# vsergeev/luaradio

Hardware: NVIDIA H100
Metric: WBFM-mono chain Msamples/s (input samples) @N H100; FIR-128 HBM GB/s vs roofline (higher is better)
Workload: dtype f32

## Files before the change

luaradio_b200/csrc/common.cuh:

```cuda
#pragma once
#include <cuda_runtime.h>
#include <stdint.h>
#include <stddef.h>
#include <atomic>
#include <math.h>

namespace lrb {

#define LRB_MAX_DEVICES 16

struct Ctx {
    int device = -1;
    int sm_count = 132;
    cudaStream_t stream = nullptr;
    bool own_stream = false;
    std::atomic<uint64_t> launches{0};
    int reserve_ctas = 0;
    long long lead_samples = 0;
    cudaEvent_t lead_event = nullptr;
    cudaStream_t side = nullptr;
    cudaEvent_t ev_fork = nullptr, ev_join = nullptr;
};
Ctx& ctx();
void set_error(const char* fmt, ...);
bool cuda_ok(cudaError_t e, const char* what);

#define LRB_CHECK(call)                                   \
    do {                                                  \
        if (!::lrb::cuda_ok((call), #call)) return -1;    \
    } while (0)

inline uint64_t turns_to_fix(double turns) {
    long double t = (long double)turns;
    t -= floorl(t);
    long double f = ldexpl(t, 64);
    if (f >= 18446744073709551616.0L) return 0;
    return (uint64_t)f;
}

constexpr size_t SIDE_STREAM_MIN = (size_t)1 << 18;
cudaStream_t side_fork(cudaStream_t s);
void side_join(cudaStream_t s, cudaStream_t side);

inline void count_launch(int n = 1) { ctx().launches.fetch_add((uint64_t)n, std::memory_order_relaxed); }

enum FirKind { FIR_CRCF = 0, FIR_CCCF = 1, FIR_RRRF = 2, FIR_HILBERT = 3 };

int launch_fir_generic(FirKind kind, const void* x, const void* hist, const void* taps, int M, int D,
                       long long first, long long n_out, void* y, cudaStream_t s);
int launch_hist_update(const void* x, long long n, const void* hist_old, void* hist_new, int H,
                       int elem_size, cudaStream_t s);

bool poly_generic_supports(FirKind kind, int M, int D);
int launch_poly_generic(FirKind kind, const void* x, const void* hist, const void* taps_host, int M, int D,
                        long long first, long long n, long long n_out, void* y, cudaStream_t s);

int launch_rotator(const float2* x, float2* y, long long n, uint64_t turns_fix, uint64_t g0, cudaStream_t s);
int launch_discrim(const float2* x, const float2* prev, float* y, long long n, float inv_gain, cudaStream_t s);
int launch_downsample(const void* x, void* y, long long first, long long n_out, int D, int elem_size, cudaStream_t s);
int launch_cmag(const float2* x, float* y, long long n, cudaStream_t s);
int launch_c2r(const float2* x, float* y, long long n, cudaStream_t s);
int launch_copy_last(const void* x, long long n, void* dst, int elem_size, cudaStream_t s);
int launch_zero_segments(void* const* ptrs, const size_t* bytes, int count, cudaStream_t s);

struct IirScanWork {
    int* ticket = nullptr;
    int* flags = nullptr;
    void* agg = nullptr;
    void* pfx = nullptr;
    int max_tiles = 0;
    unsigned epoch = 0;
};
int iir_work_alloc(IirScanWork* w, int elem_size);
void iir_work_free(IirScanWork* w);
long long iir_max_per_launch(const IirScanWork& w);
int launch_iir1(bool complex_data, const void* x, long long n, void* y, const float* b_host, int nb, float c,
                const void* xhist_in, void* xhist_out, const void* ystate_in, void* ystate_out,
                long long first, int D, IirScanWork* w, cudaStream_t s);

int launch_iir_general(bool complex_data, const void* x, long long n, void* y, const float* b, int nb, const float* a, int na,
                       const void* xhist, const void* yhist, long long warm, cudaStream_t s);

int launch_synth_white(float2* dst, uint64_t n0, long long n, uint32_t seed, cudaStream_t s);
int launch_synth_fm(float2* dst, uint64_t n0, long long n, uint32_t seed, double rate, double carrier,
                    double deviation, float amp, float noise, cudaStream_t s);

#ifdef __CUDACC__
__device__ __forceinline__ float2 ffma2(float2 a, float2 b, float2 c) {
    return make_float2(__fmaf_rn(a.x, b.x, c.x), __fmaf_rn(a.y, b.y, c.y));
}
__device__ __forceinline__ float2 fmul2(float2 a, float2 b) { return make_float2(__fmul_rn(a.x, b.x), __fmul_rn(a.y, b.y)); }
__device__ __forceinline__ float2 fadd2(float2 a, float2 b) { return make_float2(__fadd_rn(a.x, b.x), __fadd_rn(a.y, b.y)); }
__device__ __forceinline__ float2 phasor_from_fix(uint64_t ph) {
    int t = (int)(uint32_t)(ph >> 32);
    float half_turns = (float)t * 4.656612873077393e-10f;
    float s, c;
    sincospif(half_turns, &s, &c);
    return make_float2(c, s);
}
__device__ __forceinline__ float fast_atan2f(float y, float x) {
    const float ax = fabsf(x), ay = fabsf(y);
    const float mx = fmaxf(ax, ay), mn = fminf(ax, ay);
    const float a = mx > 0.f ? __fdividef(mn, mx) : 0.f;
    const float z = a * a;
    float r = 0.0028340641874819994f;
    r = fmaf(r, z, -0.016005029901862144f);
    r = fmaf(r, z, 0.042587608098983765f);
    r = fmaf(r, z, -0.07495445758104324f);
    r = fmaf(r, z, 0.10636754333972931f);
    r = fmaf(r, z, -0.14202570915222168f);
    r = fmaf(r, z, 0.19992484152317047f);
    r = fmaf(r, z, -0.3333306610584259f);
    r = fmaf(r, z, 1.0f);
    r *= a;
    r = ay > ax ? 1.57079632679489662f - r : r;
    r = x < 0.f ? 3.14159265358979324f - r : r;
    return copysignf(r, y);
}
__device__ __forceinline__ float2 fast_atan2f_x2(float2 y, float2 x) {
    const float ax0 = fabsf(x.x), ay0 = fabsf(y.x), ax1 = fabsf(x.y), ay1 = fabsf(y.y);
    const float mx0 = fmaxf(ax0, ay0), mn0 = fminf(ax0, ay0), mx1 = fmaxf(ax1, ay1), mn1 = fminf(ax1, ay1);
    const float2 a = make_float2(mx0 > 0.f ? __fdividef(mn0, mx0) : 0.f, mx1 > 0.f ? __fdividef(mn1, mx1) : 0.f);
    const float2 z = fmul2(a, a);
    float2 r = make_float2(0.0028340641874819994f, 0.0028340641874819994f);
    r = ffma2(r, z, make_float2(-0.016005029901862144f, -0.016005029901862144f));
    r = ffma2(r, z, make_float2(0.042587608098983765f, 0.042587608098983765f));
    r = ffma2(r, z, make_float2(-0.07495445758104324f, -0.07495445758104324f));
    r = ffma2(r, z, make_float2(0.10636754333972931f, 0.10636754333972931f));
    r = ffma2(r, z, make_float2(-0.14202570915222168f, -0.14202570915222168f));
    r = ffma2(r, z, make_float2(0.19992484152317047f, 0.19992484152317047f));
    r = ffma2(r, z, make_float2(-0.3333306610584259f, -0.3333306610584259f));
    r = ffma2(r, z, make_float2(1.0f, 1.0f));
    r = fmul2(r, a);
    float r0 = ay0 > ax0 ? 1.57079632679489662f - r.x : r.x;
    float r1 = ay1 > ax1 ? 1.57079632679489662f - r.y : r.y;
    r0 = x.x < 0.f ? 3.14159265358979324f - r0 : r0;
    r1 = x.y < 0.f ? 3.14159265358979324f - r1 : r1;
    return make_float2(copysignf(r0, y.x), copysignf(r1, y.y));
}
__device__ __forceinline__ float2 cmul(float2 a, float2 b) {
    float2 t = fmul2(make_float2(-a.y, a.x), make_float2(b.y, b.y));
    return ffma2(a, make_float2(b.x, b.x), t);
}
#endif

}
```

luaradio_b200/csrc/tuner.cu:

```cuda
#include "common.cuh"
#include "blocks.h"

#include <cmath>
#include <cstdlib>
#include <cstring>
#include <new>
#include <string>
#include <type_traits>
#include <vector>

namespace lrb {

namespace {

#ifndef LRB_PT_THREADS
#define LRB_PT_THREADS 64
#define LRB_PT_R 8
#define LRB_PT_CTAS 8
#define LRB_PT_PREFETCH 9
#define LRB_PT_BATCH 7
#endif
#ifndef LRB_PT_EXPERIMENT
#define LRB_PT_EXPERIMENT 0
#endif
#ifndef LRB_PT_EARLY_REST
#define LRB_PT_EARLY_REST 0
#endif
constexpr int PT_THREADS = LRB_PT_THREADS;
constexpr int PT_R = LRB_PT_R;
constexpr int PT_TO = PT_THREADS * PT_R;
constexpr int PT_MAXTAPS = 144;
constexpr int PT_BATCH = LRB_PT_BATCH;

constexpr int PT_MAXIT = 48;
struct PolyParams {
    float hr[PT_MAXTAPS];
    float2 step[PT_MAXIT];
    uint64_t turns_fix;
    uint64_t g0;
    long long off;
    int M;
    float pole_c;
    float pole_cp[6];
};
constexpr int PT_POLE_WARM = (64 % LRB_PT_R == 0) ? 64 : ((72 % LRB_PT_R == 0) ? 72 : 4 * LRB_PT_R);
static_assert(PT_POLE_WARM % LRB_PT_R == 0 && PT_POLE_WARM % 4 == 0 && PT_POLE_WARM >= 64, "pole warm-up must cover whole threads");

template <int D, int Q>
struct PolyShape {
    static constexpr int RD = PT_R * D;
    static constexpr int T = Q * D + 1;
    static constexpr int SPAN = (PT_TO + Q - 1) * D + 1;
    static constexpr int PAIRS = (SPAN + 1) / 2;
    static constexpr int ITERS = (PAIRS + PT_THREADS - 1) / PT_THREADS;
    static constexpr int LOADED = 2 * ITERS * PT_THREADS;
    __host__ __device__ static constexpr int pad(int e) { return e + 2 * (e / RD); }
    static constexpr int ELEMS = LOADED + 2 * (LOADED / RD) + 2;
    static constexpr size_t SMEM = (size_t)ELEMS * sizeof(float2);
    static constexpr int RAW = ELEMS;
    static constexpr size_t SMEM_BULK = (size_t)(ELEMS + LOADED) * sizeof(float2);
    static constexpr int NSEG = (LOADED + RD - 1) / RD;
    static constexpr int PPS = RD / 2;
    static constexpr int RG = PT_THREADS / PPS;
    static constexpr int RITERS = (NSEG + RG - 1) / RG;
};

__device__ __forceinline__ uint32_t smem_addr(const void* p) { return (uint32_t)__cvta_generic_to_shared(p); }
__device__ __forceinline__ void mbar_init(uint64_t* bar) {
    asm volatile("mbarrier.init.shared::cta.b64 [%0], 1;\n\tfence.mbarrier_init.release.cluster;\n\t"
                 "fence.proxy.async.shared::cta;" :: "r"(smem_addr(bar)) : "memory");
}
__device__ __forceinline__ void mbar_expect_tx(uint64_t* bar, uint32_t bytes) {
    asm volatile("mbarrier.arrive.expect_tx.shared::cta.b64 _, [%0], %1;" :: "r"(smem_addr(bar)), "r"(bytes) : "memory");
}
__device__ __forceinline__ void mbar_wait(uint64_t* bar, uint32_t parity) {
    asm volatile("{\n\t.reg .pred p;\n\tLRB_WAIT_%=:\n\t"
                 "mbarrier.try_wait.parity.shared::cta.b64 p, [%0], %1;\n\t"
                 "@!p bra LRB_WAIT_%=;\n\t}" :: "r"(smem_addr(bar)), "r"(parity) : "memory");
}
__device__ __forceinline__ void fence_proxy_async() { asm volatile("fence.proxy.async.shared::cta;" ::: "memory"); }
__device__ __forceinline__ void bulk_g2s(void* dst, const void* src, uint32_t bytes, uint64_t* bar) {
    asm volatile("cp.async.bulk.shared::cluster.global.mbarrier::complete_tx::bytes [%0], [%1], %2, [%3];"
                 :: "r"(smem_addr(dst)), "l"(src), "r"(bytes), "r"(smem_addr(bar)) : "memory");
}

template <int B, int E, typename F>
__device__ __forceinline__ void static_for(F&& f) {
    if constexpr (B < E) {
        f(std::integral_constant<int, B>{});
        static_for<B + 1, E>(f);
    }
}

constexpr int DISC_OV = 4;
template <bool DISC>
struct TileStride { static constexpr int TS = DISC ? PT_TO - DISC_OV : PT_TO; };

template <int D, int Q, bool ROT, bool DISC, bool EDGE, bool REAL = false, bool POLE = false>
__global__ void __launch_bounds__(PT_THREADS, LRB_PT_CTAS)
polyphase_crcf_kernel(const float2* __restrict__ x, const float2* __restrict__ hist, long long n,
                      void* __restrict__ yv, long long n_out, const __grid_constant__ PolyParams P,
                      long long t_lo, long long t_hi,
                      const float2* __restrict__ prev_in, float2* __restrict__ prev_out, float inv_gain) {
    using S = PolyShape<D, Q>;
    static_assert(!(REAL && (ROT || DISC)), "the real-stream variant has no translator / discriminator");
    static_assert(REAL || !POLE, "the fused pole exists in the real-stream variant only");
    constexpr int PW = POLE ? PT_POLE_WARM : 0;
    constexpr int PAY = PT_TO - PW;
    constexpr int TS = REAL ? 2 * PAY : TileStride<DISC>::TS;
    constexpr int NPRE = S::ITERS < LRB_PT_PREFETCH ? S::ITERS : LRB_PT_PREFETCH;
    constexpr int LANE1 = PAY * D;
    const float* __restrict__ xr = reinterpret_cast<const float*>(x);
    const float* __restrict__ histr = reinterpret_cast<const float*>(hist);
    extern __shared__ __align__(16) float2 smem[];
    __shared__ float2 s_edge[PT_THREADS / 32];
    const int tid = threadIdx.x, lane = tid & 31, warp = tid >> 5;
    const int Hm1 = P.M - 1;

    constexpr bool BULK = !EDGE && !REAL && DISC;
    __shared__ __align__(8) uint64_t s_bar;
    uint32_t bar_phase = 0;

    float2 A0 = make_float2(1.f, 0.f), A1 = make_float2(1.f, 0.f);
    const int rg = tid / S::PPS, rw = tid - rg * S::PPS;
    constexpr int NE0 = (BULK && ROT) ? S::RITERS : 1;
    float2 E0[NE0];
    float2 W1 = make_float2(1.f, 0.f);
    if constexpr (BULK && ROT) {
        W1 = phasor_from_fix(P.turns_fix);
#pragma unroll
        for (int it = 0; it < NE0; ++it)
            E0[it] = phasor_from_fix(P.turns_fix * (uint64_t)((rg + S::RG * it) * S::RD + 2 * rw));
    } else if constexpr (ROT) {
        A0 = phasor_from_fix(P.turns_fix * (uint64_t)(2 * tid));
        A1 = phasor_from_fix(P.turns_fix * (uint64_t)(2 * tid + 1));
    }
    const bool rot_last = rg < S::RG && (rg + S::RG * (S::RITERS - 1)) * S::RD + 2 * rw < S::LOADED;
    auto tile_of = [&](long long idx) -> long long { return EDGE ? (idx < t_lo ? idx : t_hi + (idx - t_lo)) : (t_lo + idx); };
    const long long n_work = EDGE ? 0 : (t_hi - t_lo);
    long long widx = blockIdx.x;

    auto issue_tile = [&](long long idx) {
        if (tid == 0) {
            fence_proxy_async();
            mbar_expect_tx(&s_bar, (uint32_t)(S::LOADED * sizeof(float2)));
            bulk_g2s(smem + S::RAW, x + (P.off + tile_of(idx) * (long long)(TS * D)), (uint32_t)(S::LOADED * sizeof(float2)), &s_bar);
        }
    };
    if constexpr (BULK) {
        if (tid == 0) mbar_init(&s_bar);
        __syncthreads();
        if (widx < n_work) issue_tile(widx);
    }

    auto ld_pair = [&](long long Bt, int k) -> float4 {
        if constexpr (REAL) {
            const float2* pa = reinterpret_cast<const float2*>(xr + Bt) + (tid + k * PT_THREADS);
            const float2 a = __ldcs(pa), b = __ldcs(pa + LANE1 / 2);
            return make_float4(a.x, b.x, a.y, b.y);
        } else {
            return __ldcs(reinterpret_cast<const float4*>(x + Bt) + (tid + k * PT_THREADS));
        }
    };
    float4 pre[NPRE];
    constexpr int REST = (S::ITERS - NPRE) < PT_BATCH ? (S::ITERS - NPRE) : PT_BATCH;
    float4 rest[REST > 0 ? REST : 1];
    if constexpr (!EDGE && !BULK) {
        if (widx < n_work) {
            const long long Bt = P.off + tile_of(widx) * (long long)(TS * D);
#pragma unroll
            for (int k = 0; k < NPRE; ++k) pre[k] = ld_pair(Bt, k);
            if constexpr (LRB_PT_EARLY_REST) {
#pragma unroll
                for (int k = 0; k < REST; ++k) rest[k] = ld_pair(Bt, NPRE + k);
            }
        }
    }

    for (;;) {
        if constexpr (!EDGE) { if (widx >= n_work) break; }
        const long long tile = tile_of(widx);
        const long long B = P.off + tile * (long long)(TS * D);
        const long long m0 = tile * TS - (DISC ? DISC_OV : 0) - PW;

        auto stage_pair = [&](float4 v, int it) {
            const int u = tid + it * PT_THREADS;
            float2 a = make_float2(v.x, v.y), b = make_float2(v.z, v.w);
            if constexpr (ROT) {
                const float2 st = P.step[it];
                a = cmul(a, cmul(A0, st));
                b = cmul(b, cmul(A1, st));
            }
            *reinterpret_cast<float4*>(smem + S::pad(2 * u)) = make_float4(a.x, a.y, b.x, b.y);
        };
        if constexpr (BULK) {
            if (LRB_PT_EXPERIMENT != 1 || widx == blockIdx.x) {
                mbar_wait(&s_bar, bar_phase);
                bar_phase ^= 1;
                if (rg < S::RG) {
                    const float2* src = smem + S::RAW + rg * S::RD + 2 * rw;
                    float2* dst = smem + rg * (S::RD + 2) + 2 * rw;
#pragma unroll
                    for (int it = 0; it < S::RITERS; ++it) {
                        if (it == S::RITERS - 1 && !rot_last) break;
                        float4 v = *reinterpret_cast<const float4*>(src + it * S::RG * S::RD);
                        if constexpr (ROT) {
                            const float2 a = cmul(make_float2(v.x, v.y), E0[it]);
                            const float2 b = cmul(make_float2(v.z, v.w), cmul(E0[it], W1));
                            v = make_float4(a.x, a.y, b.x, b.y);
                        }
                        *reinterpret_cast<float4*>(dst + it * S::RG * (S::RD + 2)) = v;
                    }
                }
            }
        } else if constexpr (!EDGE && LRB_PT_EXPERIMENT == 1) {
            if (widx == blockIdx.x) {
#pragma unroll 1
                for (int it = 0; it < S::ITERS; ++it) stage_pair(ld_pair(B, it), it);
            }
        } else if constexpr (!EDGE) {
            if constexpr (!LRB_PT_EARLY_REST) {
#pragma unroll
                for (int k = 0; k < REST; ++k) rest[k] = ld_pair(B, NPRE + k);
            }
#pragma unroll
            for (int k = 0; k < NPRE; ++k) stage_pair(pre[k], k);
#pragma unroll
            for (int k = 0; k < REST; ++k) stage_pair(rest[k], NPRE + k);
#pragma unroll 1
            for (int it0 = NPRE + REST; it0 < S::ITERS; it0 += PT_BATCH) {
                float4 buf[PT_BATCH];
#pragma unroll
                for (int k = 0; k < PT_BATCH; ++k)
                    if (it0 + k < S::ITERS) buf[k] = ld_pair(B, it0 + k);
#pragma unroll
                for (int k = 0; k < PT_BATCH; ++k)
                    if (it0 + k < S::ITERS) stage_pair(buf[k], it0 + k);
            }
        } else {
#pragma unroll 7
            for (int it = 0; it < S::ITERS; ++it) {
                const long long i0 = B + 2LL * (tid + it * PT_THREADS);
                if constexpr (REAL) {
                    auto g = [&](long long i) -> float {
                        return (i >= 0) ? (i < n ? __ldg(xr + i) : 0.f) : ((Hm1 + i >= 0) ? __ldg(histr + (Hm1 + i)) : 0.f);
                    };
                    stage_pair(make_float4(g(i0), g(i0 + LANE1), g(i0 + 1), g(i0 + 1 + LANE1)), it);
                    continue;
                }
                const float2 a = (i0 >= 0) ? (i0 < n ? __ldg(x + i0) : make_float2(0.f, 0.f))
                                           : ((Hm1 + i0 >= 0) ? __ldg(hist + (Hm1 + i0)) : make_float2(0.f, 0.f));
                const long long i1 = i0 + 1;
                const float2 b = (i1 >= 0) ? (i1 < n ? __ldg(x + i1) : make_float2(0.f, 0.f))
                                           : ((Hm1 + i1 >= 0) ? __ldg(hist + (Hm1 + i1)) : make_float2(0.f, 0.f));
                stage_pair(make_float4(a.x, a.y, b.x, b.y), it);
            }
        }
        __syncthreads();

        if constexpr (BULK && LRB_PT_EXPERIMENT != 1) {
            if (widx + gridDim.x < n_work) issue_tile(widx + gridDim.x);
        }
        if constexpr (!EDGE && !BULK && LRB_PT_EXPERIMENT != 1) {
            const long long nidx = widx + gridDim.x;
            if (nidx < n_work) {
                const long long Bn = P.off + tile_of(nidx) * (long long)(TS * D);
#pragma unroll
                for (int k = 0; k < NPRE; ++k) pre[k] = ld_pair(Bn, k);
            }
        }

        float2 acc[PT_R];
#pragma unroll
        for (int r = 0; r < PT_R; ++r) acc[r] = make_float2(0.f, 0.f);
        const float2* tb = smem + tid * (S::RD + 2);
        static_for<0, (LRB_PT_EXPERIMENT == 2 ? 1 : PT_R + Q)>([&](auto jc) {
            constexpr int j = decltype(jc)::value;
            float2 xs[D];
            constexpr int e0 = j * D;
            if constexpr (j == PT_R + Q - 1) {
                xs[0] = tb[S::pad(e0)];
            } else {
                static_for<0, D>([&](auto pc) {
                    constexpr int pp = decltype(pc)::value;
                    constexpr int e = e0 + pp;
                    if constexpr ((e & 1) && pp >= 1) {
                    } else if constexpr (!(e & 1) && pp + 1 < D) {
                        const float4 v = *reinterpret_cast<const float4*>(tb + S::pad(e));
                        xs[pp] = make_float2(v.x, v.y);
                        xs[pp + 1] = make_float2(v.z, v.w);
                    } else {
                        xs[pp] = tb[S::pad(e)];
                    }
                });
            }
            static_for<0, PT_R>([&](auto rc) {
                constexpr int r = decltype(rc)::value;
                constexpr int qq = j - r;
                if constexpr (qq >= 0 && qq <= Q) {
                    static_for<0, D>([&](auto pc) {
                        constexpr int pp = decltype(pc)::value;
                        if constexpr (qq * D + pp < S::T) {
                            const float h = P.hr[qq * D + pp];
                            acc[r] = ffma2(xs[pp], make_float2(h, h), acc[r]);
                        }
                    });
                }
            });
        });
        if constexpr (!EDGE && !BULK && LRB_PT_EARLY_REST) {
            const long long nidx = widx + gridDim.x;
            if (nidx < n_work) {
                const long long Bn = P.off + tile_of(nidx) * (long long)(TS * D);
#pragma unroll
                for (int k = 0; k < REST; ++k) rest[k] = ld_pair(Bn, NPRE + k);
            }
        }
        if constexpr (ROT && !DISC) {
            const float2 Pt = phasor_from_fix(P.turns_fix * (P.g0 + (uint64_t)B));
#pragma unroll
            for (int r = 0; r < PT_R; ++r) acc[r] = cmul(acc[r], Pt);
        }

        const long long mbase = m0 + (long long)tid * PT_R;
        if constexpr (POLE) {
            const float c = P.pole_c;
            if (tile == 0 && tid < PW / PT_R) {
#pragma unroll
                for (int r = 0; r < PT_R; ++r) acc[r].x = 0.f;
                if (tid == PW / PT_R - 1) acc[PT_R - 1].x = __ldg(reinterpret_cast<const float*>(prev_in));
            }
#pragma unroll
            for (int r = 1; r < PT_R; ++r) acc[r] = ffma2(acc[r - 1], make_float2(c, c), acc[r]);
            float2 Bv = acc[PT_R - 1];
#pragma unroll
            for (int k = 0; k < 5; ++k) {
                const float2 o = make_float2(__shfl_up_sync(0xffffffffu, Bv.x, 1 << k), __shfl_up_sync(0xffffffffu, Bv.y, 1 << k));
                if (lane >= (1 << k)) Bv = ffma2(o, make_float2(P.pole_cp[k], P.pole_cp[k]), Bv);
            }
            if (lane == 31) s_edge[warp] = Bv;
            float2 prevB = make_float2(__shfl_up_sync(0xffffffffu, Bv.x, 1), __shfl_up_sync(0xffffffffu, Bv.y, 1));
            if (lane == 0) prevB = make_float2(0.f, 0.f);
            __syncthreads();
            float2 carryW = make_float2(0.f, 0.f);
            for (int w = 0; w < warp; ++w) carryW = ffma2(carryW, make_float2(P.pole_cp[5], P.pole_cp[5]), s_edge[w]);
            float f_lane = 1.f;
#pragma unroll
            for (int k = 0; k < 5; ++k) if (lane & (1 << k)) f_lane *= P.pole_cp[k];
            const float2 excl = ffma2(carryW, make_float2(f_lane, f_lane), prevB);
            float cpow = c;
#pragma unroll
            for (int r = 0; r < PT_R; ++r) { acc[r] = ffma2(excl, make_float2(cpow, cpow), acc[r]); cpow *= c; }
        }
        if constexpr (REAL) {
            float* y = reinterpret_cast<float*>(yv);
#pragma unroll
            for (int half = 0; half < 2; ++half) {
                const long long mb = mbase + half * PAY;
                if (POLE && tid < PW / PT_R) continue;
                float v[PT_R];
#pragma unroll
                for (int r = 0; r < PT_R; ++r) v[r] = half ? acc[r].y : acc[r].x;
                if (mb + PT_R <= n_out && ((reinterpret_cast<uintptr_t>(y + mb) & 15) == 0)) {
#pragma unroll
                    for (int r = 0; r < PT_R; r += 4)
                        __stcs(reinterpret_cast<float4*>(y + mb + r), make_float4(v[r], v[r + 1], v[r + 2], v[r + 3]));
                } else {
#pragma unroll
                    for (int r = 0; r < PT_R; ++r)
                        if (mb + r < n_out) y[mb + r] = v[r];
                }
                if constexpr (POLE) {
                    if (mb <= n_out - 1 && n_out - 1 < mb + PT_R) {
#pragma unroll
                        for (int r = 0; r < PT_R; ++r)
                            if (mb + r == n_out - 1) *reinterpret_cast<float*>(prev_out) = v[r];
                    }
                }
            }
            __syncthreads();
        } else if constexpr (!DISC) {
            float2* y = reinterpret_cast<float2*>(yv);
            if (mbase + PT_R <= n_out && ((reinterpret_cast<uintptr_t>(y + mbase) & 15) == 0)) {
                float4* y4 = reinterpret_cast<float4*>(y + mbase);
#pragma unroll
                for (int r = 0; r < PT_R; r += 2)
                    __stcs(y4 + r / 2, make_float4(acc[r].x, acc[r].y, acc[r + 1].x, acc[r + 1].y));
            } else {
#pragma unroll
                for (int r = 0; r < PT_R; ++r)
                    if (mbase + r < n_out) y[mbase + r] = acc[r];
            }
            __syncthreads();
        } else {
            float* yd = reinterpret_cast<float*>(yv);
            float2 left;
            left.x = __shfl_up_sync(0xffffffffu, acc[PT_R - 1].x, 1);
            left.y = __shfl_up_sync(0xffffffffu, acc[PT_R - 1].y, 1);
            if (lane == 31) s_edge[warp] = acc[PT_R - 1];
            __syncthreads();
            if (lane == 0 && warp > 0) left = s_edge[warp - 1];
            bool zero_prev = false;
            if (EDGE && tid == 0 && tile == 0) {
                const float2 Pt = ROT ? phasor_from_fix(P.turns_fix * (P.g0 + (uint64_t)B)) : make_float2(1.f, 0.f);
                const float2 pv = __ldg(prev_in);
                acc[DISC_OV - 1] = cmul(pv, make_float2(Pt.x, -Pt.y));
                zero_prev = pv.x == 0.f && pv.y == 0.f;
            }
            const int s0 = tid * PT_R;
            float* yt = yd + m0;
            float dout[PT_R];
#pragma unroll
            for (int r = 0; r < PT_R; r += 2) {
                const float2 c0 = acc[r], p0 = (r == 0) ? left : acc[r - 1];
                const float2 c1 = acc[r + 1], p1 = acc[r];
                const float2 t0 = ffma2(c0, make_float2(p0.x, p0.x), fmul2(make_float2(c0.y, -c0.x), make_float2(p0.y, p0.y)));
                const float2 t1 = ffma2(c1, make_float2(p1.x, p1.x), fmul2(make_float2(c1.y, -c1.x), make_float2(p1.y, p1.y)));
                const float2 ang = fast_atan2f_x2(make_float2(t0.y, t1.y), make_float2(t0.x, t1.x));
                dout[r] = ang.x * inv_gain;
                dout[r + 1] = ang.y * inv_gain;
            }
            if (EDGE && zero_prev) {
                const float2 Pt = ROT ? phasor_from_fix(P.turns_fix * (P.g0 + (uint64_t)B)) : make_float2(1.f, 0.f);
                const float2 ya = ROT ? cmul(acc[DISC_OV], Pt) : acc[DISC_OV];
                const float pz = 0.f, nz = -0.f;
                const float re = __fsub_rn(__fmul_rn(ya.x, pz), __fmul_rn(ya.y, nz));
                const float im = __fadd_rn(__fmul_rn(ya.x, nz), __fmul_rn(ya.y, pz));
                dout[DISC_OV] = atan2f(im, re) * inv_gain;
            }
            if constexpr (!EDGE) {
                if (((reinterpret_cast<uintptr_t>(yt) + DISC_OV * sizeof(float)) & 15) == 0) {
                    static_assert(DISC_OV == 4 && PT_R % 4 == 0, "thread 0 skips exactly its first float4");
#pragma unroll
                    for (int r = 0; r < PT_R; r += 4)
                        if (tid > 0 || r >= DISC_OV)
                            *reinterpret_cast<float4*>(yt + s0 + r) = make_float4(dout[r], dout[r + 1], dout[r + 2], dout[r + 3]);
                } else {
#pragma unroll
                    for (int r = 0; r < PT_R; ++r)
                        if (s0 + r >= DISC_OV) yt[s0 + r] = dout[r];
                }
            } else {
                const long long room = n_out - m0;
                const int lim = room < (long long)PT_TO ? (int)room : PT_TO;
#pragma unroll
                for (int r = 0; r < PT_R; ++r) {
                    const int sl = s0 + r;
                    if (sl >= DISC_OV && sl < lim) {
                        yt[sl] = dout[r];
                        if ((long long)sl == room - 1) {
                            const float2 Pt = ROT ? phasor_from_fix(P.turns_fix * (P.g0 + (uint64_t)B)) : make_float2(1.f, 0.f);
                            *prev_out = cmul(acc[r], Pt);
                        }
                    }
                }
            }
        }
        if constexpr (EDGE) break;
        widx += gridDim.x;
    }
}

template <int D, int Q, bool ROT, bool DISC, bool REAL = false, bool POLE = false>
int launch_shape(PolyParams P, const float* hr_base, const float2* x, const float2* hist, long long n,
                 void* y, long long first, long long n_out, const float2* prev_in, float2* prev_out, float inv_gain,
                 cudaStream_t s) {
    using S = PolyShape<D, Q>;
    static_assert(S::T <= PT_MAXTAPS, "taps table too small");
    static bool configured_dev[LRB_MAX_DEVICES] = {false};
    static int ctas_dev[LRB_MAX_DEVICES] = {0};
    bool& configured = configured_dev[ctx().device & (LRB_MAX_DEVICES - 1)];
    int& ctas_per_sm = ctas_dev[ctx().device & (LRB_MAX_DEVICES - 1)];
    auto kern_i = polyphase_crcf_kernel<D, Q, ROT, DISC, false, REAL, POLE>;
    auto kern_e = polyphase_crcf_kernel<D, Q, ROT, DISC, true, REAL, POLE>;
    constexpr size_t SMEM_I = (!REAL && DISC) ? S::SMEM_BULK : S::SMEM;
    if (!configured) {
        LRB_CHECK(cudaFuncSetAttribute(kern_i, cudaFuncAttributeMaxDynamicSharedMemorySize, (int)SMEM_I));
        LRB_CHECK(cudaFuncSetAttribute(kern_e, cudaFuncAttributeMaxDynamicSharedMemorySize, (int)S::SMEM));
        LRB_CHECK(cudaOccupancyMaxActiveBlocksPerMultiprocessor(&ctas_per_sm, kern_i, PT_THREADS, SMEM_I));
        if (ctas_per_sm < 1) ctas_per_sm = 1;
        configured = true;
    }
    constexpr int PW = POLE ? PT_POLE_WARM : 0;
    constexpr int PAY = PT_TO - PW;
    constexpr int TS = REAL ? 2 * PAY : TileStride<DISC>::TS;
    long long off = first - (DISC ? (long long)DISC_OV * D : 0) - (long long)PW * D - (long long)(Q * D - 1);
    const int shift = (int)(((off % 2) + 2) % 2);
    off -= shift;
    P.off = off;
    for (int i = 0; i < PT_MAXTAPS; ++i) {
        const int k = i - shift;
        P.hr[i] = (k >= 0 && k < Q * D) ? hr_base[k] : 0.0f;
    }
    const long long tiles = (n_out + TS - 1) / TS;
    cudaEvent_t lead_event = ctx().lead_samples > 0 ? ctx().lead_event : nullptr;
    const long long lead = lead_event ? ctx().lead_samples : 0;
    long long t_lo = 0, t_hi = 0;
    if ((reinterpret_cast<uintptr_t>(x) & (REAL ? 7 : 15)) == 0) {
        const long long step = (long long)TS * D;
        const long long need = lead - off;
        t_lo = need <= 0 ? 0 : (need + step - 1) / step;
        const long long lim = n - (long long)S::LOADED - off - (REAL ? (long long)PAY * D : 0);
        t_hi = lim < 0 ? 0 : lim / step + 1;
        if (t_hi > tiles) t_hi = tiles;
        if (DISC) {
            if (t_lo < 1) t_lo = 1;
            if (t_hi > tiles - 1) t_hi = tiles - 1;
        }
        if (t_lo > t_hi) t_lo = t_hi;
    }
    const long long n_int = t_hi - t_lo, n_edge = tiles - n_int;
    cudaStream_t side = ((n_int > 0 && n_edge > 0) || (lead_event && n_edge > 0)) ? side_fork(s) : s;
    if (n_edge > 0) {
        if (lead_event && side != s) LRB_CHECK(cudaStreamWaitEvent(side, lead_event, 0));
        else if (lead_event) LRB_CHECK(cudaStreamWaitEvent(s, lead_event, 0));
        kern_e<<<(unsigned)n_edge, PT_THREADS, S::SMEM, side>>>(x, hist, n, y, n_out, P, t_lo, t_hi, prev_in, prev_out, inv_gain);
        count_launch();
    }
    if (n_int > 0) {
        long long grid = (long long)ctx().sm_count * ctas_per_sm - ctx().reserve_ctas;
        if (grid < 1) grid = 1;
        if (grid > n_int) grid = n_int;
        kern_i<<<(unsigned)grid, PT_THREADS, SMEM_I, s>>>(x, hist, n, y, n_out, P, t_lo, t_hi, prev_in, prev_out, inv_gain);
        count_launch();
    }
    side_join(s, side);
    LRB_CHECK(cudaGetLastError());
    return 1;
}

}

struct PolyTaps {
    int M, D, Q;
    float hr[PT_MAXTAPS];
    uint64_t turns_fix;
    float2 step[PT_MAXIT];
    bool rotates = false;
    bool real_data = false;
};

static int shape_q(int M, int D, bool rotates) {
    if (D == 1 && !rotates) return M <= 16 ? 16 : (M <= 32 ? 32 : 0);
    if (D == 5 && M > 65 && M <= 128) return 26;
    return 0;
}

static int shape_q_real(int M, int D) {
    if (D == 5 && M > 130 && M <= 135) return 27;
    return 0;
}

PolyTaps* polyphase_prepare(const float* taps, int M, int D, double turns_per_sample, bool phasor_table, bool real_data) {
    int Q = real_data ? shape_q_real(M, D) : shape_q(M, D, phasor_table);
    if (!Q) return nullptr;
    PolyTaps* p = new (std::nothrow) PolyTaps();
    if (!p) return nullptr;
    p->M = M; p->D = D; p->Q = Q;
    p->real_data = real_data;
    for (int i = 0; i < PT_MAXTAPS; ++i) {
        int k = Q * D - 1 - i;
        p->hr[i] = (i < Q * D && k < M) ? taps[k] : 0.0f;
    }
    p->turns_fix = turns_to_fix(turns_per_sample);
    p->rotates = phasor_table;
    {
        const double two_pi = 6.283185307179586476925286766559;
        const long double tq = ldexpl((long double)p->turns_fix, -64);
        for (int it = 0; it < PT_MAXIT; ++it) {
            long double a = tq * (long double)(2 * PT_THREADS) * (long double)it;
            a -= floorl(a);
            p->step[it] = make_float2((float)std::cos(two_pi * (double)a), (float)std::sin(two_pi * (double)a));
        }
    }
    return p;
}

void polyphase_release(PolyTaps* p) { delete p; }

#define LRB_SHAPE_FULL(DD, QQ)                                                                                         \
    if (p->D == DD && p->Q == QQ) {                                                                                    \
        static_assert(PolyShape<DD, QQ>::ITERS <= PT_MAXIT, "step table too short");                                   \
        if (disc) return launch_shape<DD, QQ, true, true>(P, p->hr, x, hist, n, y, first, n_out, prev_in, prev_out, inv_gain, s); \
        return rot ? launch_shape<DD, QQ, true, false>(P, p->hr, x, hist, n, y, first, n_out, nullptr, nullptr, 0.f, s)    \
                   : launch_shape<DD, QQ, false, false>(P, p->hr, x, hist, n, y, first, n_out, nullptr, nullptr, 0.f, s);  \
    }
#define LRB_SHAPE_PLAIN(DD, QQ)                                                                                        \
    if (p->D == DD && p->Q == QQ && !rot && !disc) {                                                                   \
        static_assert(PolyShape<DD, QQ>::ITERS <= PT_MAXIT, "step table too short");                                   \
        return launch_shape<DD, QQ, false, false>(P, p->hr, x, hist, n, y, first, n_out, nullptr, nullptr, 0.f, s); \
    }

static int launch_polyphase_any(const PolyTaps* p, const float2* x, const float2* hist, long long n, void* y,
                                long long first, long long n_out, bool rotate, bool disc, uint64_t g0,
                                const float2* prev_in, float2* prev_out, float inv_gain, cudaStream_t s) {
    if (!p) return 0;
    if (n_out <= 0) return 1;
    const bool rot = rotate && p->rotates;
    if (disc && !rot) {
        set_error("tuner: discriminator fusion needs the translator path");
        return -1;
    }
    PolyParams P;
    std::memset(&P, 0, sizeof(P));
    P.turns_fix = p->turns_fix;
    std::memcpy(P.step, p->step, sizeof(P.step));
    P.g0 = g0;
    P.M = p->M;
    if (p->real_data) {
        if (rot || disc) { set_error("polyphase: the real-stream kernel has no translator / discriminator"); return -1; }
        const bool pole = prev_in != nullptr;
        if (pole) {
            const double c = (double)inv_gain;
            P.pole_c = inv_gain;
            double pw = std::pow(c, (double)PT_R);
            for (int k = 0; k < 6; ++k) { P.pole_cp[k] = (float)pw; pw = pw * pw; }
        }
        if (p->D == 5 && p->Q == 27)
            return pole ? launch_shape<5, 27, false, false, true, true>(P, p->hr, x, hist, n, y, first, n_out, prev_in, prev_out, 0.f, s)
                        : launch_shape<5, 27, false, false, true, false>(P, p->hr, x, hist, n, y, first, n_out, nullptr, nullptr, 0.f, s);
        return 0;
    }
    LRB_SHAPE_PLAIN(1, 16) LRB_SHAPE_PLAIN(1, 32)
    LRB_SHAPE_FULL(5, 26)
    return 0;
}

bool polyphase_pole_ok(float c) { return std::pow(std::fabs((double)c), (double)PT_POLE_WARM) <= 1e-8; }

int launch_polyphase_rrrf(const PolyTaps* p, const float* x, const float* hist, long long n, float* y,
                          long long first, long long n_out, cudaStream_t s, float pole_c, const float* z_in, float* z_out) {
    return launch_polyphase_any(p, (const float2*)x, (const float2*)hist, n, y, first, n_out, false, false, 0,
                                (const float2*)z_in, (float2*)z_out, pole_c, s);
}

int launch_polyphase_crcf(const PolyTaps* p, const float2* x, const float2* hist, long long n, float2* y,
                          long long first, long long n_out, bool rotate, uint64_t turns_fix, uint64_t g0,
                          cudaStream_t s) {
    (void)turns_fix;
    return launch_polyphase_any(p, x, hist, n, y, first, n_out, rotate, false, g0, nullptr, nullptr, 0.f, s);
}

struct TunerBlock : Block {
    int M, D;
    PolyTaps* pt = nullptr;
    void* d_hist[2] = {nullptr, nullptr};
    void* d_prev[2] = {nullptr, nullptr};
    int cur = 0, pcur = 0;
    bool disc = false;
    float gain = 1.f;
    std::string label;

    TunerBlock(PolyTaps* p, float disc_gain) : M(p->M), D(p->D), pt(p) {
        disc = disc_gain != 0.0f;
        gain = disc_gain;
        in_size = 8;
        out_size = disc ? 4 : 8;
        dev_ptrs = true;
        label = std::string(disc ? "tuner+discrim(" : "tuner(") + std::to_string(M) + ",/" + std::to_string(D) + ")";
        name = label.c_str();
    }
    ~TunerBlock() override {
        polyphase_release(pt);
        for (int i = 0; i < 2; ++i) { cudaFree(d_hist[i]); cudaFree(d_prev[i]); }
    }
    int init() override {
        size_t hb = (size_t)(M > 1 ? M - 1 : 1) * 8;
        for (int i = 0; i < 2; ++i) {
            LRB_CHECK(cudaMalloc(&d_hist[i], hb));
            LRB_CHECK(cudaMemset(d_hist[i], 0, hb));
            LRB_CHECK(cudaMalloc(&d_prev[i], 8));
            LRB_CHECK(cudaMemset(d_prev[i], 0, 8));
        }
        return 0;
    }
    size_t max_output(size_t n) const override { return n / D + 1; }
    uint64_t outputs_before(uint64_t idx) const override { return (idx + D - 1) / D; }
    long long memory_in() const override { return M - 1 + (disc ? D : 0); }
    bool supports_lead_wait() const override { return true; }
    bool state_only_on_side_stream() const override { return true; }
    void rate(unsigned* up, unsigned* down) const override { *up = 1; *down = (unsigned)D; }
    void reset_host() override { consumed = 0; cur = pcur = 0; }
    void state_buffers(std::vector<std::pair<void*, size_t>>& segs) override {
        const size_t hb = (size_t)(M > 1 ? M - 1 : 1) * 8;
        for (int i = 0; i < 2; ++i) { segs.push_back({d_hist[i], hb}); segs.push_back({d_prev[i], 8}); }
    }
    int run(const void* dx, size_t n, void* dy, size_t* n_out, cudaStream_t s) override {
        uint64_t r = consumed % (uint64_t)D;
        long long first = (long long)(((uint64_t)D - r) % (uint64_t)D);
        long long no = ((long long)n > first) ? (((long long)n - first + D - 1) / D) : 0;
        *n_out = (size_t)no;
        if (n == 0) return 0;
        cudaStream_t side = s;
        if (M > 1) {
            if (n >= SIDE_STREAM_MIN) side = side_fork(s);
            if (launch_hist_update(dx, (long long)n, d_hist[cur], d_hist[cur ^ 1], M - 1, 8, side) != 0) return -1;
        }
        int rc = launch_polyphase_any(pt, (const float2*)dx, (const float2*)d_hist[cur], (long long)n, dy, first, no, true,
                                      disc, consumed, (const float2*)d_prev[pcur], (float2*)d_prev[pcur ^ 1],
                                      disc ? 1.0f / gain : 0.f, s);
        side_join(s, side);
        if (rc <= 0) { if (rc == 0) set_error("tuner: unsupported shape"); return -1; }
        if (disc && no > 0) pcur ^= 1;
        if (M > 1) cur ^= 1;
        consumed += n;
        return 0;
    }
};

Block* make_tuner(double turns_per_sample, const float* taps, int ntaps, int decim, float disc_gain) {
    PolyTaps* p = polyphase_prepare(taps, ntaps, decim, turns_per_sample, true);
    if (!p) return nullptr;
    TunerBlock* t = new (std::nothrow) TunerBlock(p, disc_gain);
    if (!t) { polyphase_release(p); set_error("out of memory"); return nullptr; }
    if (t->init() != 0) { delete t; return nullptr; }
    return t;
}

}
```

Before: 194,300.

## Apply two-parallel fast FIR algorithm in bulk polyphase discriminator kernel

Replaces the direct polyphase FIR accumulation in the bulk discriminator path with a two-parallel fast-FIR (FFA) decomposition. Even and odd subfilters plus a summed-tap filter cut the multiply count by about a quarter. Cross-lane and cross-warp terms are fixed up through shuffles and shared memory. The tile stride shrinks by a tail of 4 outputs, and the bulk kernel's launch bound min CTAs changes to 5. This trades extra registers, some redundant computation per tile and rounding changes for fewer FMAs.

```diff
diff --git a/luaradio_b200/csrc/common.cuh b/luaradio_b200/csrc/common.cuh
--- a/luaradio_b200/csrc/common.cuh
+++ b/luaradio_b200/csrc/common.cuh
@@ -91,6 +91,7 @@
 }
 __device__ __forceinline__ float2 fmul2(float2 a, float2 b) { return make_float2(__fmul_rn(a.x, b.x), __fmul_rn(a.y, b.y)); }
 __device__ __forceinline__ float2 fadd2(float2 a, float2 b) { return make_float2(__fadd_rn(a.x, b.x), __fadd_rn(a.y, b.y)); }
+__device__ __forceinline__ float2 fsub2(float2 a, float2 b) { return make_float2(__fsub_rn(a.x, b.x), __fsub_rn(a.y, b.y)); }
 __device__ __forceinline__ float2 phasor_from_fix(uint64_t ph) {
     int t = (int)(uint32_t)(ph >> 32);
     float half_turns = (float)t * 4.656612873077393e-10f;
diff --git a/luaradio_b200/csrc/tuner.cu b/luaradio_b200/csrc/tuner.cu
--- a/luaradio_b200/csrc/tuner.cu
+++ b/luaradio_b200/csrc/tuner.cu
@@ -19,6 +19,9 @@
 #define LRB_PT_CTAS 8
 #define LRB_PT_PREFETCH 9
 #define LRB_PT_BATCH 7
+#endif
+#ifndef LRB_PT_CTAS_BULK
+#define LRB_PT_CTAS_BULK 5
 #endif
 #ifndef LRB_PT_EXPERIMENT
 #define LRB_PT_EXPERIMENT 0
@@ -35,6 +38,7 @@
 constexpr int PT_MAXIT = 48;
 struct PolyParams {
     float hr[PT_MAXTAPS];
+    float hs[PT_MAXTAPS / 2];
     float2 step[PT_MAXIT];
     uint64_t turns_fix;
     uint64_t g0;
@@ -93,11 +97,12 @@
 }
 
 constexpr int DISC_OV = 4;
+constexpr int DISC_TAIL = 4;
 template <bool DISC>
-struct TileStride { static constexpr int TS = DISC ? PT_TO - DISC_OV : PT_TO; };
+struct TileStride { static constexpr int TS = DISC ? PT_TO - DISC_OV - DISC_TAIL : PT_TO; };
 
 template <int D, int Q, bool ROT, bool DISC, bool EDGE, bool REAL = false, bool POLE = false>
-__global__ void __launch_bounds__(PT_THREADS, LRB_PT_CTAS)
+__global__ void __launch_bounds__(PT_THREADS, (!EDGE && !REAL && DISC) ? LRB_PT_CTAS_BULK : LRB_PT_CTAS)
 polyphase_crcf_kernel(const float2* __restrict__ x, const float2* __restrict__ hist, long long n,
                       void* __restrict__ yv, long long n_out, const __grid_constant__ PolyParams P,
                       long long t_lo, long long t_hi,
@@ -118,6 +123,8 @@
     const int Hm1 = P.M - 1;
 
     constexpr bool BULK = !EDGE && !REAL && DISC;
+    constexpr bool FFA = BULK && LRB_PT_EXPERIMENT != 2;
+    __shared__ float2 s_ffa[FFA ? 4 : 1][PT_THREADS / 32];
     __shared__ __align__(8) uint64_t s_bar;
     uint32_t bar_phase = 0;
 
@@ -274,9 +281,8 @@
 #pragma unroll
         for (int r = 0; r < PT_R; ++r) acc[r] = make_float2(0.f, 0.f);
         const float2* tb = smem + tid * (S::RD + 2);
-        static_for<0, (LRB_PT_EXPERIMENT == 2 ? 1 : PT_R + Q)>([&](auto jc) {
+        auto load_block = [&](auto jc, float2 (&xs)[D]) {
             constexpr int j = decltype(jc)::value;
-            float2 xs[D];
             constexpr int e0 = j * D;
             if constexpr (j == PT_R + Q - 1) {
                 xs[0] = tb[S::pad(e0)];
@@ -294,20 +300,98 @@
                     }
                 });
             }
-            static_for<0, PT_R>([&](auto rc) {
-                constexpr int r = decltype(rc)::value;
-                constexpr int qq = j - r;
-                if constexpr (qq >= 0 && qq <= Q) {
-                    static_for<0, D>([&](auto pc) {
-                        constexpr int pp = decltype(pc)::value;
-                        if constexpr (qq * D + pp < S::T) {
-                            const float h = P.hr[qq * D + pp];
-                            acc[r] = ffma2(xs[pp], make_float2(h, h), acc[r]);
+        };
+        float2 ffa_a0, ffa_fs, ffa_fb, ffa_sp;
+        const float hq = P.hr[Q * D];
+        if constexpr (FFA) {
+            static_assert(Q % 2 == 0 && PT_R % 2 == 0 && (Q / 2) * D <= PT_MAXTAPS / 2, "fast-FIR split needs even Q and R");
+            static_assert(DISC_TAIL >= 1, "the tile's last output has no A_{R/2}");
+            constexpr int QH = Q / 2, KP = PT_R / 2;
+            float2 fa[KP], fb[KP], fs[KP], uo[D], an;
+#pragma unroll
+            for (int k = 0; k < KP; ++k) fa[k] = fb[k] = fs[k] = make_float2(0.f, 0.f);
+            static_for<0, PT_R + Q>([&](auto jc) {
+                constexpr int j = decltype(jc)::value;
+                float2 xs[D];
+                load_block(jc, xs);
+                if constexpr (j == PT_R + Q - 1) {
+                } else if constexpr (j % 2 == 0) {
+                    constexpr int i = j / 2;
+                    static_for<0, KP>([&](auto kc) {
+                        constexpr int k = decltype(kc)::value, q = i - k;
+                        if constexpr (q >= 0 && q < QH) {
+                            static_for<0, D>([&](auto pc) {
+                                constexpr int pp = decltype(pc)::value;
+                                const float h = P.hr[2 * q * D + pp];
+                                fa[k] = ffma2(xs[pp], make_float2(h, h), fa[k]);
+                            });
                         }
                     });
+                    if constexpr (i >= 1 && i - 1 <= KP - 1 + QH - 1) {
+                        float2 v[D];
+#pragma unroll
+                        for (int pp = 0; pp < D; ++pp) v[pp] = fadd2(uo[pp], xs[pp]);
+                        static_for<0, KP>([&](auto kc) {
+                            constexpr int k = decltype(kc)::value, q = i - 1 - k;
+                            if constexpr (q >= 0 && q < QH) {
+                                static_for<0, D>([&](auto pc) {
+                                    constexpr int pp = decltype(pc)::value;
+                                    const float h = P.hs[q * D + pp];
+                                    fs[k] = ffma2(v[pp], make_float2(h, h), fs[k]);
+                                });
+                            }
+                        });
+                    }
+                } else {
+                    constexpr int i = (j - 1) / 2;
+                    static_for<0, KP>([&](auto kc) {
+                        constexpr int k = decltype(kc)::value, q = i - k;
+                        if constexpr (q >= 0 && q < QH) {
+                            static_for<0, D>([&](auto pc) {
+                                constexpr int pp = decltype(pc)::value;
+                                const float h = P.hr[(2 * q + 1) * D + pp];
+                                fb[k] = ffma2(xs[pp], make_float2(h, h), fb[k]);
+                            });
+                        }
+                    });
+#pragma unroll
+                    for (int pp = 0; pp < D; ++pp) uo[pp] = xs[pp];
+                }
+                if constexpr (j == 2 * QH - 1) {
+                    an = make_float2(__shfl_down_sync(0xffffffffu, fa[0].x, 1), __shfl_down_sync(0xffffffffu, fa[0].y, 1));
+                }
+                if constexpr (j >= Q) {
+                    constexpr int r = j - Q, k = r / 2;
+                    if constexpr (r % 2 == 0) {
+                        acc[r] = ffma2(xs[0], make_float2(hq, hq), fadd2(fa[k], fb[k]));
+                    } else if constexpr (k + 1 < KP) {
+                        acc[r] = ffma2(xs[0], make_float2(hq, hq), fsub2(fsub2(fs[k], fa[k + 1]), fb[k]));
+                    } else {
+                        acc[r] = ffma2(xs[0], make_float2(hq, hq), fsub2(fsub2(fs[k], an), fb[k]));
+                        ffa_a0 = fa[0]; ffa_fs = fs[k]; ffa_fb = fb[k]; ffa_sp = xs[0];
+                    }
                 }
             });
-        });
+        } else {
+            static_for<0, (LRB_PT_EXPERIMENT == 2 ? 1 : PT_R + Q)>([&](auto jc) {
+                constexpr int j = decltype(jc)::value;
+                float2 xs[D];
+                load_block(jc, xs);
+                static_for<0, PT_R>([&](auto rc) {
+                    constexpr int r = decltype(rc)::value;
+                    constexpr int qq = j - r;
+                    if constexpr (qq >= 0 && qq <= Q) {
+                        static_for<0, D>([&](auto pc) {
+                            constexpr int pp = decltype(pc)::value;
+                            if constexpr (qq * D + pp < S::T) {
+                                const float h = P.hr[qq * D + pp];
+                                acc[r] = ffma2(xs[pp], make_float2(h, h), acc[r]);
+                            }
+                        });
+                    }
+                });
+            });
+        }
         if constexpr (!EDGE && !BULK && LRB_PT_EARLY_REST) {
             const long long nidx = widx + gridDim.x;
             if (nidx < n_work) {
@@ -397,9 +481,22 @@
             float2 left;
             left.x = __shfl_up_sync(0xffffffffu, acc[PT_R - 1].x, 1);
             left.y = __shfl_up_sync(0xffffffffu, acc[PT_R - 1].y, 1);
-            if (lane == 31) s_edge[warp] = acc[PT_R - 1];
+            if constexpr (FFA) {
+                if (lane == 0) s_ffa[0][warp] = ffa_a0;
+                if (lane == 31) { s_ffa[1][warp] = ffa_fs; s_ffa[2][warp] = ffa_fb; s_ffa[3][warp] = ffa_sp; }
+            } else {
+                if (lane == 31) s_edge[warp] = acc[PT_R - 1];
+            }
             __syncthreads();
-            if (lane == 0 && warp > 0) left = s_edge[warp - 1];
+            if constexpr (FFA) {
+                auto last_out = [&](int w, float2 a) {
+                    return ffma2(s_ffa[3][w], make_float2(hq, hq), fsub2(fsub2(s_ffa[1][w], a), s_ffa[2][w]));
+                };
+                if (lane == 0 && warp > 0) left = last_out(warp - 1, ffa_a0);
+                if (lane == 31 && warp + 1 < PT_THREADS / 32) acc[PT_R - 1] = last_out(warp, s_ffa[0][warp + 1]);
+            } else {
+                if (lane == 0 && warp > 0) left = s_edge[warp - 1];
+            }
             bool zero_prev = false;
             if (EDGE && tid == 0 && tile == 0) {
                 const float2 Pt = ROT ? phasor_from_fix(P.turns_fix * (P.g0 + (uint64_t)B)) : make_float2(1.f, 0.f);
@@ -430,19 +527,20 @@
             }
             if constexpr (!EDGE) {
                 if (((reinterpret_cast<uintptr_t>(yt) + DISC_OV * sizeof(float)) & 15) == 0) {
-                    static_assert(DISC_OV == 4 && PT_R % 4 == 0, "thread 0 skips exactly its first float4");
+                    static_assert(DISC_OV == 4 && DISC_TAIL == 4 && PT_R % 4 == 0,
+                                  "thread 0 skips exactly its first float4, the last thread exactly its last");
 #pragma unroll
                     for (int r = 0; r < PT_R; r += 4)
-                        if (tid > 0 || r >= DISC_OV)
+                        if ((tid > 0 || r >= DISC_OV) && (tid < PT_THREADS - 1 || r < PT_R - DISC_TAIL))
                             *reinterpret_cast<float4*>(yt + s0 + r) = make_float4(dout[r], dout[r + 1], dout[r + 2], dout[r + 3]);
                 } else {
 #pragma unroll
                     for (int r = 0; r < PT_R; ++r)
-                        if (s0 + r >= DISC_OV) yt[s0 + r] = dout[r];
+                        if (s0 + r >= DISC_OV && s0 + r < PT_TO - DISC_TAIL) yt[s0 + r] = dout[r];
                 }
             } else {
                 const long long room = n_out - m0;
-                const int lim = room < (long long)PT_TO ? (int)room : PT_TO;
+                const int lim = room < (long long)(PT_TO - DISC_TAIL) ? (int)room : PT_TO - DISC_TAIL;
 #pragma unroll
                 for (int r = 0; r < PT_R; ++r) {
                     const int sl = s0 + r;
@@ -492,6 +590,8 @@
         const int k = i - shift;
         P.hr[i] = (k >= 0 && k < Q * D) ? hr_base[k] : 0.0f;
     }
+    for (int q = 0; 2 * q + 1 < Q; ++q)
+        for (int p = 0; p < D; ++p) P.hs[q * D + p] = P.hr[2 * q * D + p] + P.hr[(2 * q + 1) * D + p];
     const long long tiles = (n_out + TS - 1) / TS;
     cudaEvent_t lead_event = ctx().lead_samples > 0 ? ctx().lead_event : nullptr;
     const long long lead = lead_event ? ctx().lead_samples : 0;
```

New measurement: 212,300, median of 6. +9.2%, better.
